# baidu/BaikalDB

Measured on AMD Instinct MI355X. Metric: scanned rows/sec (whole node), 1e9-row filter+GROUP BY, higher is better.
Workload: dtype int64/f64; 1 GPU; config3_1e9_mixed; rows_per_gpu=1000000000, groups=1048512, rows_passed_rank0=450008433, predicates=3, group_keys=2, aggs=4

## Files before the change

### baikaldb_amd/csrc/bkdpart.inc

```

#define DPART_T 16

struct DenseSpec {
    uint64_t base0, base1;
    uint32_t k1bits;
    uint32_t span;
    uint32_t shift;
    uint32_t P;
    uint32_t hshift;
    int32_t  nv;
    int32_t  vslot[BK_MAX_AGGS];
    int32_t  vop[BK_MAX_AGGS];
};

struct DRecLayout {
    int32_t  nwords;
    int32_t  off32[BK_MAX_AGGS];
    int32_t  wide[BK_MAX_AGGS];
    uint64_t vbase[BK_MAX_AGGS];
    int32_t  pk;
    int32_t  pknf;
    uint32_t pkdidsh;
    uint32_t pksh[2];
    uint32_t pkmask[2];
// ... 33 lines not shown
        }
    } else if (c.lshift == 1) {
        uint64_t w[4];
        #pragma unroll
        for (int i = 0; i < 2; i++)
            __builtin_memcpy(&w[2 * i], p + 16 * i, 16);
        #pragma unroll
        for (int j = 0; j < 16; j++) {
            uint64_t raw = (w[j >> 2] >> ((j & 3) * 16)) & c.mask;
            o.d[j] = (uint32_t)((((uint64_t)c.base + raw) ^ flip) - sub);
        }
    } else {
        uint64_t w[2];
        __builtin_memcpy(w, p, 16);
        #pragma unroll
        for (int j = 0; j < 16; j++) {
            uint64_t raw = (w[j >> 3] >> ((j & 7) * 8)) & c.mask;
            o.d[j] = (uint32_t)((((uint64_t)c.base + raw) ^ flip) - sub);
        }
    }
    return o;
}

__device__ __forceinline__ Enc8 stage_enc8(const DevCol& c, int64_t rb,
                                           uint64_t flip, uint64_t sub) {
    Enc8 o;
    const char* p = (const char*)c.data + (rb << c.lshift);
    if (c.lshift == 2) {
        uint64_t w[4];
        #pragma unroll
        for (int i = 0; i < 2; i++)
            __builtin_memcpy(&w[2 * i], p + 16 * i, 16);
        #pragma unroll
        for (int j = 0; j < 8; j++) {
            uint64_t raw = (w[j >> 1] >> ((j & 1) * 32)) & c.mask;
            o.d[j] = (uint32_t)((((uint64_t)c.base + raw) ^ flip) - sub);
        }
    } else if (c.lshift == 1) {
        uint64_t w[2];
        __builtin_memcpy(w, p, 16);
        #pragma unroll
        for (int j = 0; j < 8; j++) {
            uint64_t raw = (w[j >> 2] >> ((j & 3) * 16)) & c.mask;
            o.d[j] = (uint32_t)((((uint64_t)c.base + raw) ^ flip) - sub);
        }
    } else {
        uint64_t w;
        __builtin_memcpy(&w, p, 8);
        #pragma unroll
        for (int j = 0; j < 8; j++) {
            uint64_t raw = (w >> (j * 8)) & c.mask;
            o.d[j] = (uint32_t)((((uint64_t)c.base + raw) ^ flip) - sub);
        }
    }
    return o;
}

__device__ __forceinline__ W8 stage_w8(const void* data, int64_t rb) {
    W8 o;
    const char* p = (const char*)data + ((uint64_t)rb << 3);
    #pragma unroll
    for (int i = 0; i < 4; i++)
        __builtin_memcpy(&o.v[2 * i], p + 16 * i, 16);
    return o;
}

__device__ __forceinline__ uint32_t conj_mask16(const BkConjunct& cj,
                                                const DevCol& c, int64_t rb) {
    const char* p = (const char*)c.data + (rb << c.lshift);
    uint32_t m = 0;
    const int64_t lit = cj.lit_i;
    const int op3 = 3 * cj.op;
    if (c.lshift == 2) {
        uint64_t w[8];
        #pragma unroll
        for (int i = 0; i < 4; i++)
            __builtin_memcpy(&w[2 * i], p + 16 * i, 16);
        #pragma unroll
        for (int j = 0; j < 16; j++) {
            int64_t v = (int64_t)((uint64_t)c.base
                                  + ((w[j >> 1] >> ((j & 1) * 32)) & c.mask));
            int cmp = (v > lit) - (v < lit);
            m |= ((0x19D2Au >> (op3 + cmp + 1)) & 1u) << j;
// ... 7 lines not shown
        for (int j = 0; j < 16; j++) {
            int64_t v = (int64_t)((uint64_t)c.base
                                  + ((w[j >> 2] >> ((j & 3) * 16)) & c.mask));
            int cmp = (v > lit) - (v < lit);
            m |= ((0x19D2Au >> (op3 + cmp + 1)) & 1u) << j;
        }
    } else {
        uint64_t w[2];
        __builtin_memcpy(w, p, 16);
        #pragma unroll
        for (int j = 0; j < 16; j++) {
            int64_t v = (int64_t)((uint64_t)c.base
                                  + ((w[j >> 3] >> ((j & 7) * 8)) & c.mask));
            int cmp = (v > lit) - (v < lit);
            m |= ((0x19D2Au >> (op3 + cmp + 1)) & 1u) << j;
        }
    }
    return m;
}

template <int BS, bool SIMPLE, bool VEC, int KV, int NCJ = 4>
__global__ void __launch_bounds__(BS)
k_dhisto(DevCols cols, BkQuerySpec q, DenseSpec ds, int64_t row_begin,
         int64_t row_end, uint16_t* passbits, uint32_t* H,
         uint64_t* rows_passed) {
    constexpr int T = DPART_T;
    extern __shared__ __attribute__((aligned(16))) uint64_t laux_[];
    uint32_t* lhist = (uint32_t*)(laux_ + 1);
    if (threadIdx.x == 0) laux_[0] = 0;
    for (uint32_t b = threadIdx.x; b < ds.P; b += BS) lhist[b] = 0;
    __syncthreads();
    int64_t gstride = (int64_t)gridDim.x * BS;
    int64_t lin = (int64_t)blockIdx.x * BS + threadIdx.x;
    int64_t my_passed = 0;
    for (int64_t b0 = row_begin + lin * T; b0 < row_end; b0 += gstride * T) {
        uint32_t pb = 0;
        if (VEC && b0 + T <= row_end) {
            pb = 0xFFFFu;
            #pragma unroll
            for (int k = 0; k < NCJ; k++) {
                if (!pb) break;
                pb &= conj_mask16(q.conjuncts[k],
                                  cols.c[q.conjuncts[k].col], b0);
            }
            if (KV >= 1 && pb) {
                const DevCol& c0 = cols.c[q.group_cols[0]];
                uint64_t flip0 = c0.type == BK_STRING ? 0 : (1ull << 63);
// ... 29 lines not shown
                m &= m - 1;
                int64_t r = b0 + j;
                uint32_t b;
                if (ds.hshift != 0xFFFFFFFFu) {
                    const DevCol& c0 = cols.c[q.group_cols[0]];
                    uint64_t d0 = (SIMPLE ? enc_value_nf(c0, r)
                                          : enc_value(c0, r)) - ds.base0;
                    b = (uint32_t)(d0 >> ds.hshift);
                } else {
                    b = dense_did<SIMPLE>(cols, q, ds, r) >> ds.shift;
                }
                atomicAdd(&lhist[b], 1u);
            }
        }
    }
    long long wsum = my_passed;
    for (int off = 32; off > 0; off >>= 1) wsum += __shfl_down(wsum, off, 64);
    if ((threadIdx.x & 63) == 0)
        atomicAdd((unsigned long long*)&laux_[0], (unsigned long long)wsum);
    __syncthreads();
    if (threadIdx.x == 0)
        atomicAdd((unsigned long long*)rows_passed,
                  (unsigned long long)laux_[0]);
    for (uint32_t b = threadIdx.x; b < ds.P; b += BS)
        H[(size_t)blockIdx.x * ds.P + b] = lhist[b];
}

__device__ __forceinline__ void drec_put(uint64_t* regs, int off32, int wide,
                                         uint64_t v) {
    if (wide) {
        regs[off32 >> 1] = v;
    } else if (off32 & 1) {
        regs[off32 >> 1] |= v << 32;
    } else {
        regs[off32 >> 1] |= v & 0xFFFFFFFFull;
    }
}
__device__ __forceinline__ uint64_t drec_get(const uint64_t* my, int off32,
                                             int wide) {
    uint64_t w = my[off32 >> 1];
    if (wide) return w;
    return (off32 & 1) ? (w >> 32) : (w & 0xFFFFFFFFull);
}

template <bool SIMPLE>
__device__ __forceinline__ void dscatter_row(
        const DevCols& cols, const BkQuerySpec& q, const DenseSpec& ds,
        const DRecLayout& lay, int64_t r, uint32_t* lcur, uint64_t* rec) {
// ... 13 lines not shown
                else f = (uint64_t)v.i - (lay.wide[a] ? 0 : lay.vbase[a]);
                break;
            case BK_AGG_AVG:
                memcpy(&f, &v.d, 8);
                break;
            case BK_AGG_MIN:
            case BK_AGG_MAX:
                f = agg_enc(cols, as, q.agg_in_types[a], v, r)
                    - (lay.wide[a] ? 0 : lay.vbase[a]);
                break;
            default: break;
        }
        drec_put(regs, lay.off32[a], lay.wide[a], f);
    }
    uint32_t b = did >> ds.shift;
    uint32_t pos = atomicAdd(&lcur[b], 1u);
    scatter_store_rec(rec + (size_t)pos * lay.nwords, regs, lay.nwords);
}

template <int BS, bool SIMPLE>
__global__ void __launch_bounds__(BS)
k_dscatter(DevCols cols, BkQuerySpec q, DenseSpec ds, DRecLayout lay,
           int64_t row_begin, int64_t row_end, const uint16_t* passbits,
           const uint32_t* H, uint64_t* rec) {
    constexpr int T = DPART_T;
    extern __shared__ __attribute__((aligned(16))) uint64_t lmem[];
    uint32_t* lcur = (uint32_t*)lmem;
    for (uint32_t b = threadIdx.x; b < ds.P; b += BS)
        lcur[b] = H[(size_t)blockIdx.x * ds.P + b];
    __syncthreads();
    int64_t gstride = (int64_t)gridDim.x * BS;
    int64_t lin = (int64_t)blockIdx.x * BS + threadIdx.x;
    for (int64_t b0 = row_begin + lin * T; b0 < row_end; b0 += gstride * T) {
        uint32_t m = passbits[(b0 - row_begin) / T];
        while (m) {
            int j = __builtin_ctz(m);
            m &= m - 1;
            dscatter_row<SIMPLE>(cols, q, ds, lay, b0 + j, lcur, rec);
        }
    }
}

__device__ __forceinline__ void dagg_apply(const BkQuerySpec& q,
                                           const DRecLayout& lay, int32_t a,
                                           uint64_t f, uint64_t* lv) {
    switch (q.aggs[a].agg_type) {
        case BK_AGG_SUM:
            if (q.agg_in_types[a] == BK_DOUBLE) {
                double dd;
                memcpy(&dd, &f, 8);
                atomic_add_f64_lds(lv, dd);
            } else {
// ... 54 lines not shown
        } else {
            f = pay[wi++];
        }
        dagg_apply(q, lay, a, f, &lval[(size_t)l * nv + ds.vslot[a]]);
    }
}

struct DScatE {
    int32_t  ncol[2];
    uint64_t nflip[2];
    uint64_t nsub[2];
    int32_t  wcol[3];
    int32_t  wmode[3];
    int32_t  naslot[2];
    int32_t  nop[2];
    int32_t  waslot[3];
    int32_t  wop[3];
};

template <int BS, int NK, int NAR, int NF, bool ABS = false, bool PK = false>
__global__ void __launch_bounds__(BS)
k_dscatter_e(DevCols cols, BkQuerySpec q, DenseSpec ds, DRecLayout lay,
             DScatE prm, int64_t row_begin, int64_t row_end,
             const uint16_t* passbits, const uint32_t* H, uint64_t* rec,
             uint32_t* hdr, uint32_t hb, uint64_t* vslab, uint32_t* tslab) {
    constexpr int T = DPART_T;
    constexpr int NU32 = 1 + NAR;
    constexpr int WOFF = (NU32 + 1) / 2;
    constexpr int NWORDS = NF > 0 ? WOFF + NF : (NU32 + 1) / 2;
    extern __shared__ __attribute__((aligned(16))) uint64_t lmem[];
    const uint32_t win = ABS ? 1u << ds.shift : 0;
    const int nv = ds.nv;
    uint64_t* lval = lmem;
    uint32_t* ltou = (uint32_t*)(lmem + (ABS ? (size_t)win * nv : 0));
    uint32_t* lcur = ABS ? ltou + win : (uint32_t*)lmem;
    if (ABS) {
        for (uint32_t i = threadIdx.x; i < win * (uint32_t)nv; i += BS)
            lval[i] = 0;
        for (uint32_t i = threadIdx.x; i < win; i += BS) ltou[i] = 0;
    }
    for (uint32_t b = threadIdx.x; b < ds.P; b += BS)
        lcur[b] = H[(size_t)blockIdx.x * ds.P + b];
    __syncthreads();
    int64_t gstride = (int64_t)gridDim.x * BS;
    int64_t lin = (int64_t)blockIdx.x * BS + threadIdx.x;
    for (int64_t b0 = row_begin + lin * T; b0 < row_end; b0 += gstride * T) {
        uint32_t pb = passbits[(b0 - row_begin) / T];
        if (!pb) continue;
        if (b0 + T > row_end) {
            while (pb) {
                int j = __builtin_ctz(pb);
                pb &= pb - 1;
                int64_t r = b0 + j;
                const DevCol& c0 = cols.c[q.group_cols[0]];
                uint64_t flip0 = c0.type == BK_STRING ? 0 : (1ull << 63);
                uint64_t d0 = (((uint64_t)cell_i64(c0, r)) ^ flip0)
                              - ds.base0;
                uint32_t did;
                if (NK == 1) {
                    did = (uint32_t)d0;
                } else {
                    const DevCol& c1 = cols.c[q.group_cols[1]];
                    uint64_t flip1 = c1.type == BK_STRING ? 0 : (1ull << 63);
                    uint64_t d1 = (((uint64_t)cell_i64(c1, r)) ^ flip1)
                                  - ds.base1;
                    did = (uint32_t)((d0 << ds.k1bits) | d1);
                }
                uint64_t regs[NWORDS];
                #pragma unroll
                for (int w = 0; w < NWORDS; w++) regs[w] = 0;
                regs[0] = did;
                #pragma unroll
// ... 30 lines not shown
                    #pragma unroll
                    for (int i = 0; i < NAR; i++) {
                        uint64_t w = regs[(1 + i) >> 1];
                        uint32_t f = (uint32_t)(((1 + i) & 1) ? (w >> 32)
                                                              : w);
                        hw |= (f & lay.pkmask[i]) << lay.pksh[i];
                    }
                    hdr[pos] = hw;
                    #pragma unroll
                    for (int i = 0; i < NF; i++)
                        rec[(size_t)pos * NF + i] = regs[WOFF + i];
                } else {
                    uint64_t* dst = rec + (size_t)pos * NWORDS;
                    #pragma unroll
                    for (int w = 0; w < NWORDS; w++) dst[w] = regs[w];
                }
            }
            continue;
        }
        #pragma unroll
        for (int h = 0; h < 2; h++) {
            uint32_t sub8 = (pb >> (8 * h)) & 0xFFu;
            if (!sub8) continue;
            int64_t rb = b0 + 8 * h;
            const DevCol& c0 = cols.c[q.group_cols[0]];
            uint64_t flip0 = c0.type == BK_STRING ? 0 : (1ull << 63);
            Enc8 dd = stage_enc8(c0, rb, flip0, ds.base0);
            if (NK == 2) {
                const DevCol& c1 = cols.c[q.group_cols[1]];
                uint64_t flip1 = c1.type == BK_STRING ? 0 : (1ull << 63);
                Enc8 d1 = stage_enc8(c1, rb, flip1, ds.base1);
                #pragma unroll
                for (int j = 0; j < 8; j++)
                    dd.d[j] = (dd.d[j] << ds.k1bits) | d1.d[j];
            }
            Enc8 nf[NAR > 0 ? NAR : 1];
            #pragma unroll
            for (int i = 0; i < NAR; i++)
                nf[i] = stage_enc8(cols.c[prm.ncol[i]], rb, prm.nflip[i],
                                   prm.nsub[i]);
            W8 wf[NF > 0 ? NF : 1];
            #pragma unroll
            for (int i = 0; i < NF; i++)
                wf[i] = stage_w8(cols.c[prm.wcol[i]].data, rb);
            #pragma unroll
            for (int j = 0; j < 8; j++) {
                if (!((sub8 >> j) & 1u)) continue;
                uint32_t did = dd.d[j];
                uint64_t wv[NF > 0 ? NF : 1];
                #pragma unroll
                for (int i = 0; i < NF; i++) {
                    uint64_t raw = wf[i].v[j];
                    uint64_t v = raw;
                    if (prm.wmode[i] == 1) v = raw ^ (1ull << 63);
                    else if (prm.wmode[i] == 2)
                        v = raw ^ ((uint64_t)((int64_t)raw >> 63)
                                   | 0x8000000000000000ull);
                    else if (prm.wmode[i] == 3) {
                        double dc = (double)(int64_t)raw;
                        memcpy(&v, &dc, 8);
                    }
                    wv[i] = v;
                }
                if (ABS && did - hb < win) {
                    uint32_t rel = did - hb;
                    atomicAdd(&ltou[rel], 1u);
                    uint32_t bse = rel * (uint32_t)(NAR + NF);
// ... 250 lines not shown
    }
}


static int ceil_log2_u64(uint64_t x) {
    int b = 0;
    while ((1ull << b) < x && b < 63) b++;
    return b;
}

typedef decltype(&k_dhisto<512, false, false, 0>) DHistoFn;
typedef decltype(&k_dscatter<512, false>) DScatFn;
typedef decltype(&k_dscatter_e<512, 1, 0, 0, false>) DScatEFn;
typedef decltype(&k_dagg<1024, 1>) DAggFn;

struct DensePlan {
    int pref;
    DenseSpec ds;
    DRecLayout lay;
    bool simple;
    BkQuerySpec qpad;
    const BkQuerySpec* qk;
    int nblocks, threads;
    uint32_t nch;
    DHistoFn histo_fn;
    DScatFn scat_fn;
    DScatEFn scat_e, scat_abs;
    DScatE eprm;
    DAggFn dagg_fn;
    size_t histo_lds, scat_lds, abs_lds, dagg_lds;
    bool dabs_on;
    double dabs_min;
    size_t abs_win;
    int pipe;
    uint64_t dagg_chunk;
    uint32_t dagg_grid;
    DensePlan() = default;
    DensePlan(const DensePlan&) = delete;
};

static bool dense_spans(BkgTable* t, const BkQuerySpec* q, DenseSpec* ds,
                        uint64_t* span_out) {
    if (q->n_group < 1 || q->n_group > 2) return false;
    if (any_group_bits(q)) return false;
    for (int32_t k = 0; k < q->n_group; k++) {
        if (q->group_fns[k]) return false;
        if (t->valid[q->group_cols[k]]) return false;
// ... 189 lines not shown
    lay->pknf = nf;
    lay->pkdidsh = (uint32_t)tot;
    lay->pksh[0] = nar == 2 ? (uint32_t)bits[1] : 0;
    lay->pksh[1] = 0;
    for (int i = 0; i < 2; i++)
        lay->pkmask[i] = bits[i] >= 32 ? 0xFFFFFFFFu : ((1u << bits[i]) - 1u);
    return true;
}

static bool dense_plan(DensePlan* pl, BkgTable* t, const BkQuerySpec* q) {
    pl->pref = 1;
    if (const char* e = getenv("BK_DENSE")) pl->pref = atoi(e);
    if (pl->pref == 0) return false;
    DenseSpec& ds = pl->ds;
    uint64_t span = 0;
    if (!dense_spans(t, q, &ds, &span) ||
        !dense_rec_layout(t, q, &ds, &pl->lay) ||
        !dense_bucket_shift(&ds, span))
        return false;

    pl->nblocks = 4096;
    if (const char* e = getenv("BK_DPART_BLOCKS")) pl->nblocks = atoi(e);
    if (pl->nblocks < 1) pl->nblocks = 4096;
    pl->nch = (uint32_t)((pl->nblocks + OFFS_CHUNK - 1) / OFFS_CHUNK);
    pl->threads = 512;
    DevCols dc = table_cols(t);

    const bool simple = pl->simple =
        query_simple(t, q) && getenv("BK_NO_SIMPLE") == nullptr;
    pl->qk = q;
    if (simple) { pl->qpad = pad_simple_q(q); pl->qk = &pl->qpad; }
    bool vec = simple;
    if (vec)
        for (int j = 0; j < 4; j++)
            if (dc.c[pl->qpad.conjuncts[j].col].lshift > 2) vec = false;
    int kv = 0;
    if (vec) {
        const DevCol& c0 = dc.c[q->group_cols[0]];
        bool k0ok = c0.lshift <= 2 && c0.type != BK_DOUBLE;
        if (ds.hshift != 0xFFFFFFFFu) {
            kv = k0ok ? 1 : 0;
        } else if (q->n_group >= 2) {
            const DevCol& c1 = dc.c[q->group_cols[1]];
            kv = (k0ok && c1.lshift <= 2 && c1.type != BK_DOUBLE) ? 2 : 0;
        }
    }
    bool cj2 = q->n_conjuncts <= 2;
// ... 41 lines not shown
    if (const char* e = getenv("BK_DAGG_GRID")) {
        uint32_t g = (uint32_t)atoi(e);
        if (g > 0 && g < pl->dagg_grid) pl->dagg_grid = g;
    }
    pl->pipe = 0;
    if (const char* e = getenv("BK_DPIPE"))
        pl->pipe = std::min(4, std::max(1, atoi(e)));
    return true;
}

static int run_dense(BkgAggOut* o, BkgTable* t, const BkQuerySpec* q,
                     const DensePlan& pl, int64_t row_begin, int64_t row_end) {
    const DenseSpec& ds = pl.ds;
    const DRecLayout& lay = pl.lay;
    int64_t range = row_end - row_begin;
    if (range >= (int64_t)UINT32_MAX * DPART_T) {
        set_err("dense range too large");
        return -1;
    }
    int npipe = pl.pipe ? pl.pipe : range >= 400 * 1000 * 1000 ? 2 : 1;
    ChunkSplit sp(row_begin, row_end, npipe);
    if (sp.piped() && !sp.streams) return -1;
    DevCols dc = table_cols(t);
    const uint32_t P = ds.P, nch = pl.nch;
    const int nblocks = pl.nblocks, threads = pl.threads;
    const uint64_t span_alloc = (uint64_t)P << ds.shift;

    struct Slot : ChunkBufs {
        uint16_t* passbits = nullptr;
        DDesc* ddesc = nullptr;
        uint64_t* vslab = nullptr;
        uint32_t* tslab = nullptr;
        void recycle() { ChunkBufs::recycle(); pool_free(ddesc); ddesc = nullptr; }
    } sl[2];
    uint64_t *gvals = nullptr, *gtouch = nullptr;
    auto cleanup = [&]() {
        for (Slot& s : sl) {
            pool_free(s.passbits); pool_free(s.ddesc); pool_free(s.vslab);
            pool_free(s.tslab); s.release();
        }
        pool_free(gvals); pool_free(gtouch);
    };
    uint64_t per_tiles = (uint64_t)((sp.per + DPART_T - 1) / DPART_T);
    for (int i = 0; i < sp.nslots(); i++) {
        CHK("dense", pool_alloc((void**)&sl[i].passbits, per_tiles * 2 + 16));
        CHK("dense", sl[i].alloc_prefix(nblocks, P, nch));
    }
    const size_t gvals_bytes = (size_t)span_alloc * ds.nv * 8 + 8;
    CHK("dense", pool_alloc((void**)&gvals, gvals_bytes));
    CHK("dense", pool_alloc((void**)&gtouch, (size_t)span_alloc * 8));
    CHK("dense", hipMemset(gvals, 0, gvals_bytes));
    CHK("dense", hipMemset(gtouch, 0, (size_t)span_alloc * 8));

    static const char* DNAMES[] = {"dhisto", "dtotals", "dscan", "doffs",
                                   "dscatter", "dagg", "dtotab"};
    ChunkClock ck{sp};
    CHK("dense", ck.start());
    ck.mark();
    std::vector<DDesc> descs;
    std::vector<uint32_t> h_tot(P), h_base(P);
    for (int c = 0; c < npipe; c++) {
        Chunk k;
        CHK("dense", chunk_open(sp, c, sl, &k));
        if (k.ce <= k.cb) break;
        Slot& s = sl[k.si];
        hipStream_t st = k.st;
        CHK("dense", hipMemsetAsync(s.totals, 0, (size_t)P * 4, st));
        hipLaunchKernelGGL(pl.histo_fn, dim3(nblocks), dim3(threads),
                           pl.histo_lds, st, dc, *pl.qk, ds, k.cb, k.ce,
                           s.passbits, s.H, o->ctrs + 1);
        ck.mark();
        uint64_t total = 0;
        CHK("dense", prefix_pass(s, nblocks, P, nch, st, ck, &total,
                                 h_tot.data(), h_base.data()));
        const uint32_t hotb = (uint32_t)(
            std::max_element(h_tot.begin(), h_tot.end()) - h_tot.begin());
        bool absorb = pl.dabs_on && total > 0 &&
                      h_tot[hotb] >= (uint64_t)(pl.dabs_min * (double)total);
        uint32_t* hdrp = nullptr;
        if (total > 0) {
            size_t rec_bytes = lay.pk
                ? (size_t)total * ((size_t)lay.pknf * 8 + 4) + 8
                : (size_t)total * lay.nwords * 8;
            CHK("dense", pool_alloc((void**)&s.rec, rec_bytes));
            if (lay.pk) hdrp = (uint32_t*)(s.rec + (size_t)total * lay.pknf);
            if (absorb) {
                const size_t slab = (size_t)nblocks * pl.abs_win;
                if (!s.vslab && ds.nv > 0)
                    CHK("dense", pool_alloc((void**)&s.vslab, slab * ds.nv * 8));
                if (!s.tslab)
                    CHK("dense", pool_alloc((void**)&s.tslab, slab * 4));
                hipLaunchKernelGGL(pl.scat_abs, dim3(nblocks), dim3(threads),
                                   pl.abs_lds, st, dc, *pl.qk, ds, lay,
                                   pl.eprm, k.cb, k.ce, s.passbits, s.H, s.rec,
                                   nullptr, hotb << ds.shift, s.vslab, s.tslab);
                hipLaunchKernelGGL(k_dabs_reduce, dim3(256), dim3(256), 0, st,
                                   ds, hotb << ds.shift, (uint32_t)nblocks,
                                   s.vslab, s.tslab, gvals, gtouch);
            } else if (pl.scat_e)
                hipLaunchKernelGGL(pl.scat_e, dim3(nblocks), dim3(threads),
                                   pl.scat_lds, st, dc, *pl.qk, ds, lay,
                                   pl.eprm, k.cb, k.ce, s.passbits, s.H, s.rec,
                                   hdrp, 0u, nullptr, nullptr);
            else
                hipLaunchKernelGGL(pl.scat_fn, dim3(nblocks), dim3(threads),
                                   pl.scat_lds, st, dc, *pl.qk, ds, lay, k.cb,
                                   k.ce, s.passbits, s.H, s.rec);
        }
        ck.mark();
        uint64_t CH = pl.dagg_chunk ? pl.dagg_chunk
                                    : std::max<uint64_t>(65536, total / 768);
        descs.clear();
        for (uint32_t b = 0; b < P; b++) {
            if (absorb && b == hotb) continue;
            uint64_t n = h_tot[b], s0 = h_base[b];
            for (uint64_t ofs = 0; ofs < n; ofs += CH)
                descs.push_back({b, (uint32_t)std::min<uint64_t>(CH, n - ofs),
                                 s0 + ofs});
        }
        if (total > 0 && !descs.empty()) {
            const size_t dbytes = descs.size() * sizeof(DDesc);
            CHK("dense", pool_alloc((void**)&s.ddesc, dbytes));
            CHK("dense", hipMemcpyAsync(s.ddesc, descs.data(), dbytes,
                                        hipMemcpyHostToDevice, st));
            uint32_t grid =
                (uint32_t)std::min<size_t>(descs.size(), pl.dagg_grid);
            hipLaunchKernelGGL(pl.dagg_fn, dim3(grid), dim3(1024), pl.dagg_lds,
                               st, *q, ds, lay, s.rec, hdrp, s.ddesc,
                               (uint32_t)descs.size(), gvals, gtouch);
        }
// ... 78 lines not shown
```

### baikaldb_amd/csrc/bkgpu.hip

```cpp

#include <hip/hip_runtime.h>
#include <cstdio>
#include <cstdlib>
#include <cstring>
#include <string>
#include <vector>
#include <algorithm>
#include <chrono>
#include <map>
#include <mutex>

#include "../../include/bk_common.h"
#include "../../include/bk_datagen.h"
#include "../../include/bk_keyenc.h"
#include "../../include/bk_keylayout.h"
#include "../../include/bkgpu.h"


static thread_local char g_err[512] = "";
static void set_err(const char* msg) { snprintf(g_err, sizeof g_err, "%s", msg); }
extern "C" const char* bkgpu_last_error(void) { return g_err; }

#define HIP_CHECK(x) do { hipError_t _e = (x); if (_e != hipSuccess) { \
    snprintf(g_err, sizeof g_err, "%s:%d %s: %s", __FILE__, __LINE__, #x, \
// ... 1073 lines not shown
            if (slot) {
                agg_update_slot<true>(slot, q, cols, r);
                bucketid[i] = (uint16_t)BK_HOT_BUCKET;
                return;
            }
        }
    }
    uint32_t b = PART_BUCKET(key_hash(flag, k0, k1), P);
    bucketid[i] = (uint16_t)b;
    atomicAdd(&lhist[b], 1u);
}

#define BK_PART_ROWS(BODY)                                                   \
    int64_t gstride = (int64_t)gridDim.x * blockDim.x;                       \
    for (int64_t r = row_begin + (int64_t)blockIdx.x * blockDim.x            \
                     + threadIdx.x;                                          \
         r < row_end; r += gstride) {                                        \
        BODY;                                                                \
    }

template <int BS, bool HOT, bool SIMPLE = false>
__global__ void __launch_bounds__(BS)
k_part_histo(DevCols cols, BkQuerySpec q, int64_t row_begin, int64_t row_end,
             uint32_t P, uint16_t* bucketid, uint32_t* H,
             uint64_t* gtable, uint64_t gmask, uint64_t fill_cap, uint64_t* fill,
             uint64_t* rows_passed, uint32_t* err, uint32_t lds_slots,
             uint32_t lcap, uint32_t hot_probe, uint32_t hot_min) {
    extern __shared__ __attribute__((aligned(16))) uint64_t ltab[];
    const int stride = SLOT_HDR + 2 * q.n_aggs;
    const uint32_t tslots = HOT ? lds_slots : 0;
    uint64_t* laux = ltab + (size_t)tslots * stride;
    uint32_t* lfill = (uint32_t*)&laux[0];
    uint32_t* lctr = (uint32_t*)&laux[2];
    volatile uint32_t* lmode = (volatile uint32_t*)&laux[3];
    uint32_t* lhist = (uint32_t*)&laux[4];
    for (uint32_t w = threadIdx.x; w < tslots * (uint32_t)stride + 4;
         w += blockDim.x)
        ltab[w] = 0;
    for (uint32_t b = threadIdx.x; b < P; b += blockDim.x) lhist[b] = 0;
    __syncthreads();
    const uint32_t lmask = tslots - 1;
    int64_t my_passed = 0;
    BK_PART_ROWS(
        (histo_row<BS, HOT, SIMPLE>(cols, q, r, row_begin, bucketid, P, lhist,
                            ltab, lmask, stride, lfill, lctr, lmode, lcap,
                            hot_probe, hot_min, my_passed)))
    long long w = my_passed;
    for (int off = 32; off > 0; off >>= 1) w += __shfl_down(w, off, 64);
    if ((threadIdx.x & 63) == 0)
        atomicAdd((unsigned long long*)&laux[1], (unsigned long long)w);
    __syncthreads();
    if (threadIdx.x == 0)
        atomicAdd((unsigned long long*)rows_passed, (unsigned long long)laux[1]);
    for (uint32_t b = threadIdx.x; b < P; b += blockDim.x)
        H[(size_t)blockIdx.x * P + b] = lhist[b];
    if (HOT) {
        __syncthreads();
        for (uint32_t sl = threadIdx.x; sl < tslots; sl += blockDim.x) {
            uint64_t* s = ltab + (uint64_t)sl * stride;
            if (((uint32_t*)s)[0] != 2u) continue;
            uint64_t* g = gtable_claim(gtable, gmask, stride, ((uint32_t*)s)[1],
                                       s[1], s[2], fill, fill_cap, err);
            if (!g) break;
            agg_merge_slot<false>(g, s + SLOT_HDR, q);
        }
    }
}

#define OFFS_CHUNK 128u
__global__ void k_part_totals(const uint32_t* H, uint32_t nblocks, uint32_t P,
                              uint32_t* S, uint32_t* totals) {
    uint32_t nchunks = (nblocks + OFFS_CHUNK - 1) / OFFS_CHUNK;
    uint32_t idx = blockIdx.x * blockDim.x + threadIdx.x;
    if (idx >= P * nchunks) return;
    uint32_t b = idx % P, chunk = idx / P;
    uint32_t b1 = (chunk + 1) * OFFS_CHUNK;
    if (b1 > nblocks) b1 = nblocks;
    uint32_t s = 0;
    for (uint32_t blk = chunk * OFFS_CHUNK; blk < b1; blk++)
        s += H[(size_t)blk * P + b];
    S[(size_t)chunk * P + b] = s;
    atomicAdd(&totals[b], s);
}

__global__ void __launch_bounds__(1024)
k_part_scan(const uint32_t* totals, uint32_t P, uint32_t* base,
            uint64_t* total_out) {
    __shared__ uint32_t part[1024];
    uint32_t T = blockDim.x;
    uint32_t per = (P + T - 1) / T;
    uint32_t lo = threadIdx.x * per, hi = lo + per;
    if (hi > P) hi = P;
    uint32_t s = 0;
    for (uint32_t b = lo; b < hi; b++) s += totals[b];
    part[threadIdx.x] = s;
    __syncthreads();
    for (uint32_t off = 1; off < T; off <<= 1) {
        uint32_t v = threadIdx.x >= off ? part[threadIdx.x - off] : 0;
        __syncthreads();
        part[threadIdx.x] += v;
        __syncthreads();
    }
    uint32_t run = threadIdx.x ? part[threadIdx.x - 1] : 0;
    for (uint32_t b = lo; b < hi; b++) {
        base[b] = run;
        run += totals[b];
    }
    if (threadIdx.x == T - 1 && total_out) *total_out = part[T - 1];
}

__global__ void k_part_offsets(uint32_t* H, uint32_t nblocks, uint32_t P,
                               const uint32_t* base, const uint32_t* S) {
    uint32_t nchunks = (nblocks + OFFS_CHUNK - 1) / OFFS_CHUNK;
    uint32_t idx = blockIdx.x * blockDim.x + threadIdx.x;
    if (idx >= P * nchunks) return;
    uint32_t b = idx % P, chunk = idx / P;
    uint32_t run = base[b];
    for (uint32_t c = 0; c < chunk; c++) run += S[(size_t)c * P + b];
    uint32_t b1 = (chunk + 1) * OFFS_CHUNK;
    if (b1 > nblocks) b1 = nblocks;
    for (uint32_t blk = chunk * OFFS_CHUNK; blk < b1; blk++) {
        uint32_t t = H[(size_t)blk * P + b];
        H[(size_t)blk * P + b] = run;
        run += t;
    }
}

__device__ __forceinline__ void scatter_store_rec(uint64_t* dst,
                                                  const uint64_t* regs,
                                                  int nwords) {
    typedef long long ll2 __attribute__((ext_vector_type(2)));
    #pragma unroll
    for (int w = 0; w < 8; w += 2) {
        if (w + 1 < nwords) {
            ll2 v2;
            v2.x = (long long)regs[w];
            v2.y = (long long)regs[w + 1];
            *(ll2*)&dst[w] = v2;
        } else if (w < nwords) {
            dst[w] = regs[w];
        }
    }
}

__device__ __forceinline__ void build_record(
        const DevCols& cols, const BkQuerySpec& q, const RecLayout& lay,
        int64_t r, const KeyPack& kp, uint64_t* regs) {
    uint64_t meta = kp.flag;
// ... 81 lines not shown
                uint64_t* sl = stash + (size_t)b * lay.nwords;
                #pragma unroll
                for (int w = 0; w < 8; w++)
                    prev[w] = w < lay.nwords ? sl[w] : 0;
                __hip_atomic_store(&bstate[b], 0u, __ATOMIC_RELEASE, WGP);
                uint32_t pos = atomicAdd(&lcur[b], 2u);
                uint64_t* dst = rec + (size_t)pos * lay.nwords;
                scatter_store_rec(dst, prev, lay.nwords);
                scatter_store_rec(dst + lay.nwords, regs, lay.nwords);
                done = true;
            }
        }
    }
    if (!done) {
        uint32_t pos = atomicAdd(&lcur[b], 1u);
        scatter_store_rec(rec + (size_t)pos * lay.nwords, regs, lay.nwords);
    }
}

template <int BS, bool SIMPLE = false>
__global__ void __launch_bounds__(BS)
k_part_scatter(DevCols cols, BkQuerySpec q, RecLayout lay, int64_t row_begin,
               int64_t row_end, uint32_t P, const uint16_t* bucketid,
               const uint32_t* H, uint64_t* rec, uint64_t total, int paired) {
    extern __shared__ __attribute__((aligned(16))) uint64_t lmem[];
    uint64_t* stash = lmem;
    uint32_t* lcur = (uint32_t*)(lmem + (paired ? (size_t)P * lay.nwords : 0));
    uint32_t* bstate = lcur + P;
    for (uint32_t b = threadIdx.x; b < P; b += blockDim.x) {
        lcur[b] = H[(size_t)blockIdx.x * P + b];
        if (paired) bstate[b] = 0;
    }
    __syncthreads();
    BK_PART_ROWS(
        (scatter_row<BS, SIMPLE>(cols, q, lay, r, row_begin, bucketid, lcur,
                         bstate, stash, rec, paired)))
    if (paired) {
        __syncthreads();
        for (uint32_t b = threadIdx.x; b < P; b += blockDim.x) {
            if (bstate[b] != 2u) continue;
            uint64_t* sl = stash + (size_t)b * lay.nwords;
            uint32_t pos = lcur[b]++;
            scatter_store_rec(rec + (size_t)pos * lay.nwords, sl, lay.nwords);
        }
    }
}

template <bool LDS>
__device__ __forceinline__ void agg_update_slot_rec(uint64_t* st, const BkQuerySpec& q,
                                                    const RecLayout& lay,
                                                    const uint64_t* my,
                                                    uint64_t meta) {
    for (int32_t a = 0; a < q.n_aggs; a++) {
// ... 1248 lines not shown
        return ilp == 2 ? k_part_agg<1024, 2> : k_part_agg<1024, 1>;
    return ilp == 2 ? k_part_agg<256, 2> : k_part_agg<256, 1>;
}


#define CHK(route, x) do { hipError_t e_ = (x); if (e_ != hipSuccess) { \
    snprintf(g_err, sizeof g_err, route " %s:%d %s", __FILE__, __LINE__, \
             hipGetErrorString(e_)); \
    (void)hipGetLastError(); \
    (void)hipDeviceSynchronize(); cleanup(); return -1; } } while (0)

struct ChunkSplit {
    int64_t row_begin, row_end, per;
    int npipe;
    hipStream_t* streams;
    ChunkSplit(int64_t rb, int64_t re, int n)
        : row_begin(rb), row_end(re), per((re - rb + n - 1) / n), npipe(n),
          streams(n > 1 ? pipe_streams() : nullptr) {}
    bool piped() const { return npipe > 1; }
    int nslots() const { return piped() ? 2 : 1; }
};

struct ChunkBufs {
    uint32_t *H = nullptr, *totals = nullptr, *base = nullptr, *S = nullptr;
    uint64_t *total_dev = nullptr, *rec = nullptr;
    hipError_t alloc_prefix(int nblocks, uint32_t P, uint32_t nch) {
        hipError_t e = pool_alloc((void**)&H, (size_t)nblocks * P * 4);
        if (!e) e = pool_alloc((void**)&totals, (size_t)P * 4);
        if (!e) e = pool_alloc((void**)&base, (size_t)P * 4);
        if (!e) e = pool_alloc((void**)&S, (size_t)nch * P * 4);
        if (!e) e = pool_alloc((void**)&total_dev, 8);
        return e;
    }
    void recycle() { pool_free(rec); rec = nullptr; }
    void release() {
        pool_free(H); pool_free(totals); pool_free(base); pool_free(S);
        pool_free(total_dev); pool_free(rec);
    }
};

struct Chunk { int64_t cb, ce; int si; hipStream_t st; };
template <class Slot>
static hipError_t chunk_open(const ChunkSplit& sp, int c, Slot* sl, Chunk* k) {
    k->si = sp.piped() ? (c & 1) : 0;
    k->st = sp.piped() ? sp.streams[k->si] : 0;
    k->cb = sp.row_begin + (int64_t)c * sp.per;
    k->ce = std::min(k->cb + sp.per, sp.row_end);
    if (c < 2 || k->ce <= k->cb) return hipSuccess;
    hipError_t e = hipStreamSynchronize(k->st);
    if (!e) sl[k->si].recycle();
    return e;
}

struct ChunkClock {
    const ChunkSplit& sp;
    EvTimer tm;
    double t0 = 0;
    hipError_t start() {
        hipError_t e = sp.piped() ? hipDeviceSynchronize() : hipSuccess;
        t0 = now_ms();
        return e;
    }
    void mark() { if (!sp.piped()) tm.record(); }
    hipError_t finish(BkgAggOut* o, const char* const* names,
                      const char* wall_name) {
        if (!sp.piped()) { tm.finish(o, names); return hipSuccess; }
        hipError_t e = hipStreamSynchronize(sp.streams[0]);
        if (!e) e = hipStreamSynchronize(sp.streams[1]);
        o->kernel_ms = o->t_ms[0] = (float)(now_ms() - t0);
        o->n_kernels = 1;
        snprintf(o->k_names[0], 16, "%s", wall_name);
        return e;
    }
};

static hipError_t prefix_pass(const ChunkBufs& b, int nblocks, uint32_t P,
                              uint32_t nch, hipStream_t st, ChunkClock& ck,
                              uint64_t* total, uint32_t* h_tot = nullptr,
                              uint32_t* h_base = nullptr) {
    const dim3 tiles((P * nch + 255) / 256);
    hipLaunchKernelGGL(k_part_totals, tiles, dim3(256), 0, st, b.H, nblocks,
                       P, b.S, b.totals);
    ck.mark();
    hipLaunchKernelGGL(k_part_scan, dim3(1), dim3(1024), 0, st, b.totals, P,
                       b.base, b.total_dev);
    ck.mark();
    const hipMemcpyKind D2H = hipMemcpyDeviceToHost;
    hipError_t e = hipGetLastError();
    if (!e) e = hipMemcpyAsync(total, b.total_dev, 8, D2H, st);
    if (!e && h_tot) e = hipMemcpyAsync(h_tot, b.totals, (size_t)P * 4, D2H, st);
    if (!e && h_base) e = hipMemcpyAsync(h_base, b.base, (size_t)P * 4, D2H, st);
    if (!e) e = hipStreamSynchronize(st);
    if (e) return e;
    hipLaunchKernelGGL(k_part_offsets, tiles, dim3(256), 0, st, b.H, nblocks,
                       P, b.base, b.S);
    ck.mark();
    return hipSuccess;
}

#include "bkdpart.inc"

struct PartPlan {
    uint32_t P;
    int nblocks, threads;
    uint32_t nch;
    RecLayout lay;
    bool simple;
    BkQuerySpec qpad;
    const BkQuerySpec* qk;
    HistoFn histo_fn;
    ScatFn scat_fn;
    uint32_t hot_slots, hot_cap, hot_probe, hot_min;
    size_t histo_lds;
    bool pair;
    PartAggFn agg_fn;
    int at;
    uint32_t agg_lds_slots;
    size_t agg_lds_bytes;
    uint64_t agg_chunk;
    int pipe;
    uint64_t pipe_agg_grid;
    PartPlan() = default;
    PartPlan(const PartPlan&) = delete;
};

static void part_plan(PartPlan* pl, BkgTable* t, const BkQuerySpec* q,
                      int64_t expected_groups) {
    const int stride = SLOT_HDR + 2 * q->n_aggs;
    build_rec_layout(t, q, &pl->lay);
    pl->P = 64;
    while ((int64_t)pl->P < expected_groups / 1024 && pl->P < 4096) pl->P <<= 1;
    if (const char* e = getenv("BK_PART_P")) pl->P = (uint32_t)atoi(e);
    pl->nblocks = 8192;
    if (const char* e = getenv("BK_PART_BLOCKS")) pl->nblocks = atoi(e);
    if (pl->nblocks < 1) pl->nblocks = 8192;
    pl->nch = (uint32_t)((pl->nblocks + OFFS_CHUNK - 1) / OFFS_CHUNK);
    pl->threads = 512;
    if (const char* e = getenv("BK_PART_THREADS")) pl->threads = atoi(e);
    if (pl->threads != 512 && pl->threads != 1024) pl->threads = 256;

    size_t hot_lds_cap = 50 * 1024;
    if (const char* e = getenv("BK_HOT_LDS_KB")) hot_lds_cap = (size_t)atoi(e) * 1024;
    pl->hot_slots = 512;
    if (const char* e = getenv("BK_HOT_SLOTS")) pl->hot_slots = (uint32_t)atoi(e);
    while ((size_t)pl->hot_slots * stride * 8 > hot_lds_cap) pl->hot_slots >>= 1;
    pl->hot_cap = pl->hot_slots / 2u;
    if (const char* e = getenv("BK_HOT_CAP")) pl->hot_cap = (uint32_t)atoi(e);
    if (pl->hot_cap > pl->hot_slots - pl->hot_slots / 8u)
        pl->hot_cap = pl->hot_slots - pl->hot_slots / 8u;
    pl->hot_probe = 4;
    if (const char* e = getenv("BK_HOT_PROBE")) pl->hot_probe = (uint32_t)atoi(e);
    pl->hot_min = 4097;
    if (const char* e = getenv("BK_HOT_MIN")) pl->hot_min = (uint32_t)atoi(e);
    const bool hot = pl->hot_min <= 4096;
    if (!hot) pl->hot_slots = 0;
    pl->simple = query_simple(t, q) && getenv("BK_NO_SIMPLE") == nullptr;
    pl->qk = q;
    if (pl->simple) { pl->qpad = pad_simple_q(q); pl->qk = &pl->qpad; }
    pl->histo_fn = pick_histo(pl->threads, hot, pl->simple);
// ... 19 lines not shown
    pl->pipe = -1;
    if (const char* e = getenv("BK_PIPE")) pl->pipe = std::max(0, atoi(e));
    pl->pipe_agg_grid = 32768;
    if (const char* e = getenv("BK_PIPE_AGG_GRID")) pl->pipe_agg_grid = (uint64_t)atoll(e);
}

static int run_partitioned(BkgAggOut* o, BkgTable* t, const BkQuerySpec* q,
                           int64_t row_begin, int64_t row_end,
                           int64_t expected_groups) {
    const int64_t range = row_end - row_begin;
    PartPlan pl;
    part_plan(&pl, t, q, expected_groups);
    int npipe = (range >= 400 * 1000 * 1000 &&
                 expected_groups >= (1 << 20)) ? 2 : 1;
    if (pl.pipe >= 0) npipe = pl.pipe;
    if (npipe < 2 || range < (int64_t)4 * npipe) npipe = 1;
    ChunkSplit sp(row_begin, row_end, npipe);
    const bool piped = sp.piped();
    if (piped && !sp.streams) return -1;
    if (sp.per >= (int64_t)UINT32_MAX) {
        set_err("row chunk too large for one pass");
        return -1;
    }
    const uint32_t P = pl.P, nch = pl.nch;
    const int nblocks = pl.nblocks, threads = pl.threads;

    struct Slot : ChunkBufs { uint16_t* bucketid = nullptr; } sl[2];
    auto cleanup = [&]() {
        for (Slot& s : sl) { pool_free(s.bucketid); s.release(); }
    };
    for (int i = 0; i < sp.nslots(); i++) {
        CHK("part", pool_alloc((void**)&sl[i].bucketid, (size_t)sp.per * 2));
        CHK("part", sl[i].alloc_prefix(nblocks, P, nch));
    }
    DevCols dc = table_cols(t);

    static const char* NAMES[] = {"histo", "totals", "scan", "offsets",
                                  "scatter", "part_agg"};
    ChunkClock ck{sp};
    CHK("part", ck.start());
    for (int c = 0; c < npipe; c++) {
        Chunk k;
        CHK("part", chunk_open(sp, c, sl, &k));
        if (k.ce <= k.cb) break;
        Slot& s = sl[k.si];
        hipStream_t st = k.st;
        CHK("part", hipMemsetAsync(s.totals, 0, (size_t)P * 4, st));
        ck.mark();
        hipLaunchKernelGGL(pl.histo_fn, dim3(nblocks), dim3(threads),
                           pl.histo_lds, st, dc, *pl.qk, k.cb, k.ce, P,
                           s.bucketid, s.H, o->table, o->nslots - 1,
                           (o->nslots * 7) / 8, o->ctrs, o->ctrs + 1, o->err,
                           pl.hot_slots, pl.hot_cap, pl.hot_probe, pl.hot_min);
        ck.mark();
        uint64_t total = 0;
        CHK("part", prefix_pass(s, nblocks, P, nch, st, ck, &total));
        if (!piped && debug_timing()) {
            uint64_t passed = 0;
            (void)hipMemcpy(&passed, o->ctrs + 1, 8, hipMemcpyDeviceToHost);
            fprintf(stderr, "[bkgpu] passed=%llu cold_records=%llu hot_absorbed=%.1f%%\n",
                    (unsigned long long)passed, (unsigned long long)total,
                    passed ? 100.0 * (double)(passed - total) / (double)passed : 0.0);
        }
        if (total > 0) {
            size_t rec_bytes = (size_t)total * pl.lay.nwords * 8;
            CHK("part", pool_alloc((void**)&s.rec, rec_bytes));
            size_t pair_lds = (size_t)P * pl.lay.nwords * 8 + (size_t)P * 8;
            int paired = !piped && pl.pair && pair_lds <= 130 * 1024;
            size_t sc_lds = paired ? pair_lds : (size_t)P * 8;
            hipLaunchKernelGGL(pl.scat_fn, dim3(nblocks), dim3(threads), sc_lds,
                               st, dc, *pl.qk, pl.lay, k.cb, k.ce, P, s.bucketid,
                               s.H, s.rec, total, paired);
        }
        ck.mark();
        if (total > 0) {
            uint64_t chunk = pl.agg_chunk ? pl.agg_chunk
                : std::max<uint64_t>(32768,
                                     std::min<uint64_t>(1u << 20, total / 4096));
            uint64_t nrec_chunks = (total + chunk - 1) / chunk;
            uint32_t grid = (uint32_t)std::min<uint64_t>(
                nrec_chunks, piped ? pl.pipe_agg_grid : 32768);
            hipLaunchKernelGGL(pl.agg_fn, dim3(grid), dim3(pl.at),
                               pl.agg_lds_bytes, st, *q, pl.lay, s.rec, total,
                               chunk, o->table, o->nslots - 1,
                               (o->nslots * 7) / 8, o->ctrs, o->err,
                               pl.agg_lds_slots);
        }
        ck.mark();
        CHK("part", hipGetLastError());
    }
    CHK("part", ck.finish(o, NAMES, "pipeline"));
    cleanup();
    return 0;
}

// ... 619 lines not shown
```

Baseline: 53.49 billion rows/s.

## Replace per-block prefix offset kernels with atomic reservation and coalesce passbit reads

After: 60.68 billion rows/s, median of 6. +13.4%, better.

```diff
diff --git a/baikaldb_amd/csrc/bkdpart.inc b/baikaldb_amd/csrc/bkdpart.inc
--- a/baikaldb_amd/csrc/bkdpart.inc
+++ b/baikaldb_amd/csrc/bkdpart.inc
@@ -79,10 +79,12 @@
     return o;
 }
 
-__device__ __forceinline__ Enc8 stage_enc8(const DevCol& c, int64_t rb,
-                                           uint64_t flip, uint64_t sub) {
+__device__ __forceinline__ Enc8 stage_enc8(const DevCol& c, int64_t rs,
+                                           uint32_t vo, uint64_t flip,
+                                           uint64_t sub) {
     Enc8 o;
-    const char* p = (const char*)c.data + (rb << c.lshift);
+    const char* p = (const char*)c.data + (rs << c.lshift)
+                    + (size_t)(vo << c.lshift);
     if (c.lshift == 2) {
         uint64_t w[4];
         #pragma unroll
@@ -113,9 +115,10 @@
     return o;
 }
 
-__device__ __forceinline__ W8 stage_w8(const void* data, int64_t rb) {
+__device__ __forceinline__ W8 stage_w8(const void* data, int64_t rs,
+                                       uint32_t vo) {
     W8 o;
-    const char* p = (const char*)data + ((uint64_t)rb << 3);
+    const char* p = (const char*)data + ((uint64_t)rs << 3) + (size_t)(vo << 3);
     #pragma unroll
     for (int i = 0; i < 4; i++)
         __builtin_memcpy(&o.v[2 * i], p + 16 * i, 16);
@@ -169,7 +172,7 @@
 template <int BS, bool SIMPLE, bool VEC, int KV, int NCJ = 4>
 __global__ void __launch_bounds__(BS)
 k_dhisto(DevCols cols, BkQuerySpec q, DenseSpec ds, int64_t row_begin,
-         int64_t row_end, uint16_t* passbits, uint32_t* H,
+         int64_t row_end, uint16_t* passbits, uint32_t* H, uint32_t* totals,
          uint64_t* rows_passed) {
     constexpr int T = DPART_T;
     extern __shared__ __attribute__((aligned(16))) uint64_t laux_[];
@@ -245,8 +248,11 @@
     if (threadIdx.x == 0)
         atomicAdd((unsigned long long*)rows_passed,
                   (unsigned long long)laux_[0]);
-    for (uint32_t b = threadIdx.x; b < ds.P; b += BS)
-        H[(size_t)blockIdx.x * ds.P + b] = lhist[b];
+    for (uint32_t b = threadIdx.x; b < ds.P; b += BS) {
+        uint32_t n = lhist[b];
+        H[(size_t)blockIdx.x * ds.P + b] = n;
+        if (n) atomicAdd(&totals[b], n);
+    }
 }
 
 __device__ __forceinline__ void drec_put(uint64_t* regs, int off32, int wide,
@@ -306,12 +312,12 @@
 __global__ void __launch_bounds__(BS)
 k_dscatter(DevCols cols, BkQuerySpec q, DenseSpec ds, DRecLayout lay,
            int64_t row_begin, int64_t row_end, const uint16_t* passbits,
-           const uint32_t* H, uint64_t* rec) {
+           const uint32_t* H, uint32_t* base, uint64_t* rec) {
     constexpr int T = DPART_T;
     extern __shared__ __attribute__((aligned(16))) uint64_t lmem[];
     uint32_t* lcur = (uint32_t*)lmem;
     for (uint32_t b = threadIdx.x; b < ds.P; b += BS)
-        lcur[b] = H[(size_t)blockIdx.x * ds.P + b];
+        lcur[b] = part_reserve(H, base, ds.P, b);
     __syncthreads();
     int64_t gstride = (int64_t)gridDim.x * BS;
     int64_t lin = (int64_t)blockIdx.x * BS + threadIdx.x;
@@ -412,8 +418,8 @@
 __global__ void __launch_bounds__(BS)
 k_dscatter_e(DevCols cols, BkQuerySpec q, DenseSpec ds, DRecLayout lay,
              DScatE prm, int64_t row_begin, int64_t row_end,
-             const uint16_t* passbits, const uint32_t* H, uint64_t* rec,
-             uint32_t* hdr, uint32_t hb, uint64_t* vslab, uint32_t* tslab) {
+             const uint16_t* passbits, const uint32_t* H, uint32_t* base,
+             uint64_t* rec, uint32_t* hdr, uint32_t hb, uint64_t* vslab, uint32_t* tslab) {
     constexpr int T = DPART_T;
     constexpr int NU32 = 1 + NAR;
     constexpr int WOFF = (NU32 + 1) / 2;
@@ -430,14 +436,26 @@
         for (uint32_t i = threadIdx.x; i < win; i += BS) ltou[i] = 0;
     }
     for (uint32_t b = threadIdx.x; b < ds.P; b += BS)
-        lcur[b] = H[(size_t)blockIdx.x * ds.P + b];
+        lcur[b] = part_reserve(H, base, ds.P, b);
     __syncthreads();
     int64_t gstride = (int64_t)gridDim.x * BS;
-    int64_t lin = (int64_t)blockIdx.x * BS + threadIdx.x;
-    for (int64_t b0 = row_begin + lin * T; b0 < row_end; b0 += gstride * T) {
-        uint32_t pb = passbits[(b0 - row_begin) / T];
+    const uint32_t lane = threadIdx.x & 63u;
+    const int64_t wlin = (int64_t)blockIdx.x * BS +
+        (__builtin_amdgcn_readfirstlane((int)threadIdx.x) & ~63);
+    for (int64_t wb = row_begin + wlin * T; wb < row_end; wb += gstride * T) {
+        const bool whole = wb + 64 * T <= row_end;
+        uint32_t pb;
+        if (whole) {
+            const uint8_t* pby =
+                (const uint8_t*)passbits + (wb - row_begin) / 8;
+            pb = (uint32_t)pby[lane] | ((uint32_t)pby[64 + lane] << 8);
+        } else {
+            if (wb + lane * T >= row_end) continue;
+            pb = passbits[(wb - row_begin) / T + lane];
+        }
         if (!pb) continue;
-        if (b0 + T > row_end) {
+        if (!whole && wb + lane * T + T > row_end) {
+            const int64_t b0 = wb + lane * T;
             while (pb) {
                 int j = __builtin_ctz(pb);
                 pb &= pb - 1;
@@ -514,14 +532,15 @@
         for (int h = 0; h < 2; h++) {
             uint32_t sub8 = (pb >> (8 * h)) & 0xFFu;
             if (!sub8) continue;
-            int64_t rb = b0 + 8 * h;
+            const uint32_t vo = whole ? 8 * (64 * h + lane)
+                                      : T * lane + 8 * h;
             const DevCol& c0 = cols.c[q.group_cols[0]];
             uint64_t flip0 = c0.type == BK_STRING ? 0 : (1ull << 63);
-            Enc8 dd = stage_enc8(c0, rb, flip0, ds.base0);
+            Enc8 dd = stage_enc8(c0, wb, vo, flip0, ds.base0);
             if (NK == 2) {
                 const DevCol& c1 = cols.c[q.group_cols[1]];
                 uint64_t flip1 = c1.type == BK_STRING ? 0 : (1ull << 63);
-                Enc8 d1 = stage_enc8(c1, rb, flip1, ds.base1);
+                Enc8 d1 = stage_enc8(c1, wb, vo, flip1, ds.base1);
                 #pragma unroll
                 for (int j = 0; j < 8; j++)
                     dd.d[j] = (dd.d[j] << ds.k1bits) | d1.d[j];
@@ -529,12 +548,12 @@
             Enc8 nf[NAR > 0 ? NAR : 1];
             #pragma unroll
             for (int i = 0; i < NAR; i++)
-                nf[i] = stage_enc8(cols.c[prm.ncol[i]], rb, prm.nflip[i],
+                nf[i] = stage_enc8(cols.c[prm.ncol[i]], wb, vo, prm.nflip[i],
                                    prm.nsub[i]);
             W8 wf[NF > 0 ? NF : 1];
             #pragma unroll
             for (int i = 0; i < NF; i++)
-                wf[i] = stage_w8(cols.c[prm.wcol[i]].data, rb);
+                wf[i] = stage_w8(cols.c[prm.wcol[i]].data, wb, vo);
             #pragma unroll
             for (int j = 0; j < 8; j++) {
                 if (!((sub8 >> j) & 1u)) continue;
@@ -831,7 +850,6 @@
     BkQuerySpec qpad;
     const BkQuerySpec* qk;
     int nblocks, threads;
-    uint32_t nch;
     DHistoFn histo_fn;
     DScatFn scat_fn;
     DScatEFn scat_e, scat_abs;
@@ -1067,7 +1085,6 @@
     pl->nblocks = 4096;
     if (const char* e = getenv("BK_DPART_BLOCKS")) pl->nblocks = atoi(e);
     if (pl->nblocks < 1) pl->nblocks = 4096;
-    pl->nch = (uint32_t)((pl->nblocks + OFFS_CHUNK - 1) / OFFS_CHUNK);
     pl->threads = 512;
     DevCols dc = table_cols(t);
 
@@ -1155,7 +1172,7 @@
     ChunkSplit sp(row_begin, row_end, npipe);
     if (sp.piped() && !sp.streams) return -1;
     DevCols dc = table_cols(t);
-    const uint32_t P = ds.P, nch = pl.nch;
+    const uint32_t P = ds.P;
     const int nblocks = pl.nblocks, threads = pl.threads;
     const uint64_t span_alloc = (uint64_t)P << ds.shift;
 
@@ -1177,7 +1194,7 @@
     uint64_t per_tiles = (uint64_t)((sp.per + DPART_T - 1) / DPART_T);
     for (int i = 0; i < sp.nslots(); i++) {
         CHK("dense", pool_alloc((void**)&sl[i].passbits, per_tiles * 2 + 16));
-        CHK("dense", sl[i].alloc_prefix(nblocks, P, nch));
+        CHK("dense", sl[i].alloc_prefix(nblocks, P));
     }
     const size_t gvals_bytes = (size_t)span_alloc * ds.nv * 8 + 8;
     CHK("dense", pool_alloc((void**)&gvals, gvals_bytes));
@@ -1201,10 +1218,10 @@
         CHK("dense", hipMemsetAsync(s.totals, 0, (size_t)P * 4, st));
         hipLaunchKernelGGL(pl.histo_fn, dim3(nblocks), dim3(threads),
                            pl.histo_lds, st, dc, *pl.qk, ds, k.cb, k.ce,
-                           s.passbits, s.H, o->ctrs + 1);
+                           s.passbits, s.H, s.totals, o->ctrs + 1);
         ck.mark();
         uint64_t total = 0;
-        CHK("dense", prefix_pass(s, nblocks, P, nch, st, ck, &total,
+        CHK("dense", prefix_pass(s, P, st, ck, &total,
                                  h_tot.data(), h_base.data()));
         const uint32_t hotb = (uint32_t)(
             std::max_element(h_tot.begin(), h_tot.end()) - h_tot.begin());
@@ -1225,20 +1242,20 @@
                     CHK("dense", pool_alloc((void**)&s.tslab, slab * 4));
                 hipLaunchKernelGGL(pl.scat_abs, dim3(nblocks), dim3(threads),
                                    pl.abs_lds, st, dc, *pl.qk, ds, lay,
-                                   pl.eprm, k.cb, k.ce, s.passbits, s.H, s.rec,
-                                   nullptr, hotb << ds.shift, s.vslab, s.tslab);
+                                   pl.eprm, k.cb, k.ce, s.passbits, s.H,
+                                   s.base, s.rec, nullptr, hotb << ds.shift, s.vslab, s.tslab);
                 hipLaunchKernelGGL(k_dabs_reduce, dim3(256), dim3(256), 0, st,
                                    ds, hotb << ds.shift, (uint32_t)nblocks,
                                    s.vslab, s.tslab, gvals, gtouch);
             } else if (pl.scat_e)
                 hipLaunchKernelGGL(pl.scat_e, dim3(nblocks), dim3(threads),
                                    pl.scat_lds, st, dc, *pl.qk, ds, lay,
-                                   pl.eprm, k.cb, k.ce, s.passbits, s.H, s.rec,
-                                   hdrp, 0u, nullptr, nullptr);
+                                   pl.eprm, k.cb, k.ce, s.passbits, s.H,
+                                   s.base, s.rec, hdrp, 0u, nullptr, nullptr);
             else
                 hipLaunchKernelGGL(pl.scat_fn, dim3(nblocks), dim3(threads),
                                    pl.scat_lds, st, dc, *pl.qk, ds, lay, k.cb,
-                                   k.ce, s.passbits, s.H, s.rec);
+                                   k.ce, s.passbits, s.H, s.base, s.rec);
         }
         ck.mark();
         uint64_t CH = pl.dagg_chunk ? pl.dagg_chunk
diff --git a/baikaldb_amd/csrc/bkgpu.hip b/baikaldb_amd/csrc/bkgpu.hip
--- a/baikaldb_amd/csrc/bkgpu.hip
+++ b/baikaldb_amd/csrc/bkgpu.hip
@@ -1119,7 +1119,7 @@
 template <int BS, bool HOT, bool SIMPLE = false>
 __global__ void __launch_bounds__(BS)
 k_part_histo(DevCols cols, BkQuerySpec q, int64_t row_begin, int64_t row_end,
-             uint32_t P, uint16_t* bucketid, uint32_t* H,
+             uint32_t P, uint16_t* bucketid, uint32_t* H, uint32_t* totals,
              uint64_t* gtable, uint64_t gmask, uint64_t fill_cap, uint64_t* fill,
              uint64_t* rows_passed, uint32_t* err, uint32_t lds_slots,
              uint32_t lcap, uint32_t hot_probe, uint32_t hot_min) {
@@ -1149,8 +1149,11 @@
     __syncthreads();
     if (threadIdx.x == 0)
         atomicAdd((unsigned long long*)rows_passed, (unsigned long long)laux[1]);
-    for (uint32_t b = threadIdx.x; b < P; b += blockDim.x)
-        H[(size_t)blockIdx.x * P + b] = lhist[b];
+    for (uint32_t b = threadIdx.x; b < P; b += blockDim.x) {
+        uint32_t n = lhist[b];
+        H[(size_t)blockIdx.x * P + b] = n;
+        if (n) atomicAdd(&totals[b], n);
+    }
     if (HOT) {
         __syncthreads();
         for (uint32_t sl = threadIdx.x; sl < tslots; sl += blockDim.x) {
@@ -1162,22 +1165,6 @@
             agg_merge_slot<false>(g, s + SLOT_HDR, q);
         }
     }
-}
-
-#define OFFS_CHUNK 128u
-__global__ void k_part_totals(const uint32_t* H, uint32_t nblocks, uint32_t P,
-                              uint32_t* S, uint32_t* totals) {
-    uint32_t nchunks = (nblocks + OFFS_CHUNK - 1) / OFFS_CHUNK;
-    uint32_t idx = blockIdx.x * blockDim.x + threadIdx.x;
-    if (idx >= P * nchunks) return;
-    uint32_t b = idx % P, chunk = idx / P;
-    uint32_t b1 = (chunk + 1) * OFFS_CHUNK;
-    if (b1 > nblocks) b1 = nblocks;
-    uint32_t s = 0;
-    for (uint32_t blk = chunk * OFFS_CHUNK; blk < b1; blk++)
-        s += H[(size_t)blk * P + b];
-    S[(size_t)chunk * P + b] = s;
-    atomicAdd(&totals[b], s);
 }
 
 __global__ void __launch_bounds__(1024)
@@ -1206,21 +1193,11 @@
     if (threadIdx.x == T - 1 && total_out) *total_out = part[T - 1];
 }
 
-__global__ void k_part_offsets(uint32_t* H, uint32_t nblocks, uint32_t P,
-                               const uint32_t* base, const uint32_t* S) {
-    uint32_t nchunks = (nblocks + OFFS_CHUNK - 1) / OFFS_CHUNK;
-    uint32_t idx = blockIdx.x * blockDim.x + threadIdx.x;
-    if (idx >= P * nchunks) return;
-    uint32_t b = idx % P, chunk = idx / P;
-    uint32_t run = base[b];
-    for (uint32_t c = 0; c < chunk; c++) run += S[(size_t)c * P + b];
-    uint32_t b1 = (chunk + 1) * OFFS_CHUNK;
-    if (b1 > nblocks) b1 = nblocks;
-    for (uint32_t blk = chunk * OFFS_CHUNK; blk < b1; blk++) {
-        uint32_t t = H[(size_t)blk * P + b];
-        H[(size_t)blk * P + b] = run;
-        run += t;
-    }
+__device__ __forceinline__ uint32_t part_reserve(const uint32_t* H,
+                                                 uint32_t* base, uint32_t P,
+                                                 uint32_t b) {
+    uint32_t cnt = H[(size_t)blockIdx.x * P + b];
+    return cnt ? atomicAdd(&base[b], cnt) : 0;
 }
 
 __device__ __forceinline__ void scatter_store_rec(uint64_t* dst,
@@ -1348,13 +1325,14 @@
 __global__ void __launch_bounds__(BS)
 k_part_scatter(DevCols cols, BkQuerySpec q, RecLayout lay, int64_t row_begin,
                int64_t row_end, uint32_t P, const uint16_t* bucketid,
-               const uint32_t* H, uint64_t* rec, uint64_t total, int paired) {
+               const uint32_t* H, uint32_t* base, uint64_t* rec,
+               uint64_t total, int paired) {
     extern __shared__ __attribute__((aligned(16))) uint64_t lmem[];
     uint64_t* stash = lmem;
     uint32_t* lcur = (uint32_t*)(lmem + (paired ? (size_t)P * lay.nwords : 0));
     uint32_t* bstate = lcur + P;
     for (uint32_t b = threadIdx.x; b < P; b += blockDim.x) {
-        lcur[b] = H[(size_t)blockIdx.x * P + b];
+        lcur[b] = part_reserve(H, base, P, b);
         if (paired) bstate[b] = 0;
     }
     __syncthreads();
@@ -2649,19 +2627,18 @@
 };
 
 struct ChunkBufs {
-    uint32_t *H = nullptr, *totals = nullptr, *base = nullptr, *S = nullptr;
+    uint32_t *H = nullptr, *totals = nullptr, *base = nullptr;
     uint64_t *total_dev = nullptr, *rec = nullptr;
-    hipError_t alloc_prefix(int nblocks, uint32_t P, uint32_t nch) {
+    hipError_t alloc_prefix(int nblocks, uint32_t P) {
         hipError_t e = pool_alloc((void**)&H, (size_t)nblocks * P * 4);
         if (!e) e = pool_alloc((void**)&totals, (size_t)P * 4);
         if (!e) e = pool_alloc((void**)&base, (size_t)P * 4);
-        if (!e) e = pool_alloc((void**)&S, (size_t)nch * P * 4);
         if (!e) e = pool_alloc((void**)&total_dev, 8);
         return e;
     }
     void recycle() { pool_free(rec); rec = nullptr; }
     void release() {
-        pool_free(H); pool_free(totals); pool_free(base); pool_free(S);
+        pool_free(H); pool_free(totals); pool_free(base);
         pool_free(total_dev); pool_free(rec);
     }
 };
@@ -2701,13 +2678,10 @@
     }
 };
 
-static hipError_t prefix_pass(const ChunkBufs& b, int nblocks, uint32_t P,
-                              uint32_t nch, hipStream_t st, ChunkClock& ck,
-                              uint64_t* total, uint32_t* h_tot = nullptr,
+static hipError_t prefix_pass(const ChunkBufs& b, uint32_t P, hipStream_t st,
+                              ChunkClock& ck, uint64_t* total,
+                              uint32_t* h_tot = nullptr,
                               uint32_t* h_base = nullptr) {
-    const dim3 tiles((P * nch + 255) / 256);
-    hipLaunchKernelGGL(k_part_totals, tiles, dim3(256), 0, st, b.H, nblocks,
-                       P, b.S, b.totals);
     ck.mark();
     hipLaunchKernelGGL(k_part_scan, dim3(1), dim3(1024), 0, st, b.totals, P,
                        b.base, b.total_dev);
@@ -2719,8 +2693,6 @@
     if (!e && h_base) e = hipMemcpyAsync(h_base, b.base, (size_t)P * 4, D2H, st);
     if (!e) e = hipStreamSynchronize(st);
     if (e) return e;
-    hipLaunchKernelGGL(k_part_offsets, tiles, dim3(256), 0, st, b.H, nblocks,
-                       P, b.base, b.S);
     ck.mark();
     return hipSuccess;
 }
@@ -2730,7 +2702,6 @@
 struct PartPlan {
     uint32_t P;
     int nblocks, threads;
-    uint32_t nch;
     RecLayout lay;
     bool simple;
     BkQuerySpec qpad;
@@ -2761,7 +2732,6 @@
     pl->nblocks = 8192;
     if (const char* e = getenv("BK_PART_BLOCKS")) pl->nblocks = atoi(e);
     if (pl->nblocks < 1) pl->nblocks = 8192;
-    pl->nch = (uint32_t)((pl->nblocks + OFFS_CHUNK - 1) / OFFS_CHUNK);
     pl->threads = 512;
     if (const char* e = getenv("BK_PART_THREADS")) pl->threads = atoi(e);
     if (pl->threads != 512 && pl->threads != 1024) pl->threads = 256;
@@ -2827,7 +2797,7 @@
         set_err("row chunk too large for one pass");
         return -1;
     }
-    const uint32_t P = pl.P, nch = pl.nch;
+    const uint32_t P = pl.P;
     const int nblocks = pl.nblocks, threads = pl.threads;
 
     struct Slot : ChunkBufs { uint16_t* bucketid = nullptr; } sl[2];
@@ -2836,7 +2806,7 @@
     };
     for (int i = 0; i < sp.nslots(); i++) {
         CHK("part", pool_alloc((void**)&sl[i].bucketid, (size_t)sp.per * 2));
-        CHK("part", sl[i].alloc_prefix(nblocks, P, nch));
+        CHK("part", sl[i].alloc_prefix(nblocks, P));
     }
     DevCols dc = table_cols(t);
 
@@ -2854,12 +2824,12 @@
         ck.mark();
         hipLaunchKernelGGL(pl.histo_fn, dim3(nblocks), dim3(threads),
                            pl.histo_lds, st, dc, *pl.qk, k.cb, k.ce, P,
-                           s.bucketid, s.H, o->table, o->nslots - 1,
+                           s.bucketid, s.H, s.totals, o->table, o->nslots - 1,
                            (o->nslots * 7) / 8, o->ctrs, o->ctrs + 1, o->err,
                            pl.hot_slots, pl.hot_cap, pl.hot_probe, pl.hot_min);
         ck.mark();
         uint64_t total = 0;
-        CHK("part", prefix_pass(s, nblocks, P, nch, st, ck, &total));
+        CHK("part", prefix_pass(s, P, st, ck, &total));
         if (!piped && debug_timing()) {
             uint64_t passed = 0;
             (void)hipMemcpy(&passed, o->ctrs + 1, 8, hipMemcpyDeviceToHost);
@@ -2875,7 +2845,7 @@
             size_t sc_lds = paired ? pair_lds : (size_t)P * 8;
             hipLaunchKernelGGL(pl.scat_fn, dim3(nblocks), dim3(threads), sc_lds,
                                st, dc, *pl.qk, pl.lay, k.cb, k.ce, P, s.bucketid,
-                               s.H, s.rec, total, paired);
+                               s.H, s.base, s.rec, total, paired);
         }
         ck.mark();
         if (total > 0) {
```
